# cmusphinx/pocketsphinx

Hardware: NVIDIA H100
Metric: frames/sec senone-eval+Viterbi (higher is better)
Workload: dtype f32->i16/i32

## Files before the change

pocketsphinx_b200/csrc/psb_api.cu:

```cuda
#include "psb_internal.cuh"

#include <stdarg.h>
#include <stdlib.h>
#include <string.h>

#include <algorithm>
#include <vector>

std::atomic<long long> g_psb_launches{0};
std::atomic<long long> g_psb_bytes_live{0};

static thread_local char g_err[512] = "";

void psb_set_error(const char *fmt, ...)
{
    va_list ap;
    va_start(ap, fmt);
    vsnprintf(g_err, sizeof(g_err), fmt, ap);
    va_end(ap);
}

extern "C" const char *psb_last_error(void) { return g_err; }
extern "C" int psb_abi_version(void) { return PSB_ABI_VERSION; }
extern "C" int64_t psb_kernel_launch_count(void) { return g_psb_launches.load(); }
// ... 126 lines not shown
    PSB_CUDA(cudaSetDevice(device));
    PSB_REQUIRE(!(d->fixed_point && d->kind == PSB_KIND_MS), "fixed-point arithmetic is implemented for ptm and semi-continuous models only");
    std::unique_ptr<psb_model_t> m(new psb_model_t());
    m->device = device;
    m->kind = d->kind; m->n_sen = d->n_sen; m->n_mgau = d->n_mgau; m->n_feat = d->n_feat;
    m->n_density = d->n_density; m->topn = d->topn;
    m->ds_ratio = d->ds_ratio > 0 ? d->ds_ratio : 1;
    m->aw = d->aw != 0 ? d->aw : 1;
    m->sumlen = 0;
    for (int f = 0; f < d->n_feat; ++f) {
        m->featlen[f] = d->featlen[f];
        m->featoff[f] = m->sumlen;
        m->sumlen += d->featlen[f];
    }
    m->K = m->n_mgau * m->n_feat;
    m->mixw_4bit = d->mixw_cb != nullptr;
    m->fixed_point = d->fixed_point != 0;
    m->logadd_ms_size = d->logadd_ms_size;
    m->logadd_ms_zero = d->logadd_ms_zero;
    const bool dev = d->on_device != 0;
    const cudaMemcpyKind to_dev = dev ? cudaMemcpyDeviceToDevice : cudaMemcpyHostToDevice;
    int rc = build_records(m.get(), d->mean, d->var, d->det, dev);
    if (!rc) rc = upload(m->d_featlen, m->featlen, PSB_MAX_FEAT, false);
    if (!rc) rc = upload(m->d_featoff, m->featoff, PSB_MAX_FEAT, false);
    if (rc) return rc;

    std::vector<int32_t> s2c(m->n_sen);
    if (cudaMemcpy(s2c.data(), d->sen2cb, m->n_sen * sizeof(int32_t),
                   dev ? cudaMemcpyDeviceToHost : cudaMemcpyHostToHost) != cudaSuccess) {
        psb_set_error("copying sen2cb failed");
        return PSB_ERR_CUDA;
    }
    std::vector<uint16_t> s2c16(m->n_sen);
    for (int i = 0; i < m->n_sen; ++i) {
        PSB_REQUIRE(s2c[i] >= 0 && s2c[i] < m->n_mgau, "sen2cb[%d] = %d out of range", i, s2c[i]);
        s2c16[i] = (uint16_t)s2c[i];
    }
    {
        const int nq = (m->n_sen + 3) / 4;
        std::vector<int16_t> quadcb(nq, -1);
        std::vector<int32_t> bsen;
        for (int q = 0; q < nq; ++q) {
            const int s0 = 4 * q;
            bool uni = s0 + 3 < m->n_sen && m->n_mgau <= 32767;
            for (int i = 1; uni && i < 4; ++i) uni = s2c[s0 + i] == s2c[s0];
            if (uni) quadcb[q] = (int16_t)s2c[s0];
            else for (int i = 0; i < 4 && s0 + i < m->n_sen; ++i) bsen.push_back(s0 + i);
        }
        m->n_bsen = (int)bsen.size();
        if ((rc = upload(m->d_quadcb, quadcb.data(), nq, false)) || (rc = upload(m->d_bsen, bsen.data(), bsen.size(), false)))
            return rc;
    }
    m->sen_is_cb = m->n_mgau == m->n_sen;
    for (int i = 0; m->sen_is_cb && i < m->n_sen; ++i) m->sen_is_cb = s2c[i] == i;
    if ((rc = upload(m->d_sen2cb, s2c16.data(), m->n_sen, false)) || (rc = upload(m->d_sen2cb32, s2c.data(), m->n_sen, false)))
        return rc;

    if (m->kind == PSB_KIND_MS) {
        m->mixw_row = m->n_sen;
        m->mixw_stride = m->n_sen;
        rc = upload(m->d_mixw, d->mixw, (size_t)m->n_sen * m->n_feat * m->n_density, dev);
    }
    else {
        m->mixw_row = m->mixw_4bit ? (m->n_sen + 1) / 2 : m->n_sen;
        m->mixw_stride = roundup(m->mixw_row, 128);
        const size_t rows = (size_t)m->n_feat * m->n_density;
        rc = m->d_mixw.reserve(rows * m->mixw_stride);
        if (!rc && (cudaMemset(m->d_mixw, 0, rows * m->mixw_stride) != cudaSuccess ||
                    cudaMemcpy2D(m->d_mixw, m->mixw_stride, d->mixw, m->mixw_row, m->mixw_row, rows, to_dev) != cudaSuccess)) {
            psb_set_error("uploading mixture weights failed: %s", cudaGetErrorString(cudaGetLastError()));
            rc = PSB_ERR_CUDA;
        }
    }
    if (!rc && m->mixw_4bit) rc = upload(m->d_mixw_cb, d->mixw_cb, 16, dev);
    if (!rc && d->logadd8) {
        rc = m->d_logadd8.reserve(PSB_LOGADD8_N);
        if (!rc && (cudaMemset(m->d_logadd8, 0, PSB_LOGADD8_N) != cudaSuccess ||
                    cudaMemcpy(m->d_logadd8, d->logadd8, 256, to_dev) != cudaSuccess)) {
            psb_set_error("uploading the log-add table failed: %s", cudaGetErrorString(cudaGetLastError()));
            rc = PSB_ERR_CUDA;
        }
        else if (!rc) {
            uint8_t t[256];
            if (cudaMemcpy(t, m->d_logadd8, 256, cudaMemcpyDeviceToHost) == cudaSuccess)
                for (int i = 0; i < 256; ++i) m->logadd8_max = std::max<int>(m->logadd8_max, t[i]);
        }
    }
    if (rc) return rc;
    PSB_REQUIRE(m->kind == PSB_KIND_MS || d->logadd8, "logadd8 table required for ptm/semi models");
    if (m->kind == PSB_KIND_MS) {
        PSB_REQUIRE(d->logadd_ms && d->logadd_ms_size > 0, "logadd_ms table required for ms models");
        rc = upload(m->d_logadd_ms, d->logadd_ms, (size_t)d->logadd_ms_size, dev);
        if (rc) return rc;
    }
    if (d->topn_beam) {
        uint8_t tb[PSB_MAX_FEAT] = {0};
        if (cudaMemcpy(tb, d->topn_beam, m->n_feat, dev ? cudaMemcpyDeviceToHost : cudaMemcpyHostToHost) != cudaSuccess)
            return PSB_ERR_CUDA;
        for (int f = 0; f < m->n_feat; ++f) {
            m->topn_beam[f] = tb[f];
            if (tb[f]) m->has_topn_beam = true;
        }
    }
    int32_t tb[PSB_MAX_FEAT] = {0};
    for (int f = 0; f < m->n_feat; ++f) tb[f] = m->has_topn_beam ? m->topn_beam[f] : 0;
    rc = upload(m->d_topn_beam, tb, PSB_MAX_FEAT, false);
    if (rc) return rc;
    *out = m.release();
    return PSB_OK;
}

extern "C" void psb_model_free(psb_model_t *m)
{
    if (!m) return;
    cudaSetDevice(m->device);
    delete m;
}

extern "C" int psb_model_update_gaussians(psb_model_t *m, const float *mean, const float *var, const float *det)
{
    PSB_REQUIRE(m && mean && var && det, "psb_model_update_gaussians: null argument");
    PSB_CUDA(cudaSetDevice(m->device));
    PSB_CUDA(cudaDeviceSynchronize());
    return build_records(m, mean, var, det, false);
}

extern "C" int psb_model_n_sen(const psb_model_t *m) { return m ? m->n_sen : 0; }
extern "C" int psb_model_device(const psb_model_t *m) { return m ? m->device : -1; }


extern "C" int psb_batch_create(psb_model_t *m, int32_t max_utts, int64_t max_frames, psb_batch_t **out)
{
    PSB_REQUIRE(m && out && max_utts > 0 && max_frames > 0, "psb_batch_create: bad argument");
    const char *v = getenv("PSB_TOPN_VARIANT"), *impl = getenv("PSB_TC_IMPL");
    PSB_REQUIRE(!v || !strcmp(v, "6"),
                "psb_batch_create: PSB_TOPN_VARIANT=%s; the top-N kernel now follows from the model (the only accepted value is 6)", v);
    PSB_REQUIRE(!impl || !strcmp(impl, "wgmma"), "psb_batch_create: PSB_TC_IMPL=%s; the only accepted value is wgmma", impl);
    PSB_CUDA(cudaSetDevice(m->device));
    std::unique_ptr<psb_batch_t> b(new psb_batch_t());
    b->m = m;
    b->max_utts = max_utts;
    b->max_frames = max_frames;
    {
        const char *p = getenv("PSB_PIPELINE");
        b->n_pipe = p ? atoi(p) : 0;
        if (b->n_pipe < 0) b->n_pipe = 0;
        if (b->n_pipe > 8) b->n_pipe = 8;
    }
    cudaError_t e = b->stream.create();
    for (int i = 0; i < 4 && e == cudaSuccess; ++i) e = b->ev[i].create();
    for (int i = 0; i < 2 && e == cudaSuccess; ++i) e = b->tev[i].create();
    if (e == cudaSuccess) e = b->fork_ev.create(cudaEventDisableTiming);
    if (e == cudaSuccess) e = b->join_ev.create(cudaEventDisableTiming);
    if (e != cudaSuccess) {
        psb_set_error("psb_batch_create: %s", cudaGetErrorString(e));
        return PSB_ERR_CUDA;
    }
    int rc = b->d_feats.reserve((size_t)max_frames * m->sumlen);
    if (!rc) rc = b->d_senscr.reserve((size_t)max_frames * m->n_sen);
    if (!rc && m->kind != PSB_KIND_MS) rc = b->topn.reserve((size_t)max_frames * m->K);
    if (rc) return rc;
    b->d_topn = b->topn;
    *out = b.release();
    return PSB_OK;
}

extern "C" void psb_batch_free(psb_batch_t *b)
{
// ... 270 lines not shown
```

pocketsphinx_b200/csrc/psb_internal.cuh:

```cuda
#pragma once

#include <cuda_runtime.h>
#include <stdint.h>
#include <stdio.h>

#include <atomic>
#include <memory>
#include <string>
#include <vector>

#include "../../include/psb200.h"
#include "psb_mem.cuh"

#define PSB_SENSCR_SHIFT 10
#define PSB_MAX_NEG_ASCR 96
#define PSB_TMAT_WORST (-255)
#define PSB_BAD_SSID 0xffff
#define PSB_LOGADD8_N 512

void psb_set_error(const char *fmt, ...);
extern std::atomic<long long> g_psb_launches;

__device__ __forceinline__ float2 psb_fadd2_rn(float2 a, float2 b) { return make_float2(__fadd_rn(a.x, b.x), __fadd_rn(a.y, b.y)); }
__device__ __forceinline__ float2 psb_fmul2_rn(float2 a, float2 b) { return make_float2(__fmul_rn(a.x, b.x), __fmul_rn(a.y, b.y)); }

inline int psb_sm_count(int device)
{
    int n = 1;
    cudaDeviceGetAttribute(&n, cudaDevAttrMultiProcessorCount, device);
    return n;
}

#define PSB_CUDA(call)                                                                   \
    do {                                                                                 \
        cudaError_t e__ = (call);                                                        \
        if (e__ != cudaSuccess) {                                                        \
            psb_set_error("%s:%d: %s -> %s", __FILE__, __LINE__, #call,                  \
                          cudaGetErrorString(e__));                                      \
            return PSB_ERR_CUDA;                                                         \
        }                                                                                \
    } while (0)

#define PSB_LAUNCH_CHECK()                                                               \
    do {                                                                                 \
        g_psb_launches.fetch_add(1, std::memory_order_relaxed);                          \
        cudaError_t e__ = cudaGetLastError();                                            \
        if (e__ != cudaSuccess) {                                                        \
            psb_set_error("%s:%d: kernel launch -> %s", __FILE__, __LINE__,              \
                          cudaGetErrorString(e__));                                      \
            return PSB_ERR_CUDA;                                                         \
        }                                                                                \
    } while (0)

#define PSB_REQUIRE(cond, ...)                                                           \
    do {                                                                                 \
        if (!(cond)) {                                                                   \
            psb_set_error(__VA_ARGS__);                                                  \
            return PSB_ERR_ARG;                                                          \
        }                                                                                \
    } while (0)

static inline int psb_check_utt_off(const char *fn, const int32_t *utt_off, int32_t n_utt)
{
    PSB_REQUIRE(utt_off[0] == 0, "%s: utt_off[0] must be 0", fn);
    for (int u = 0; u < n_utt; ++u)
        PSB_REQUIRE(utt_off[u + 1] >= utt_off[u], "%s: utt_off not monotone at %d", fn, u);
    return PSB_OK;
}

static inline int roundup(int x, int m) { return (x + m - 1) / m * m; }

static inline int rec_floats(int featlen) { return roundup(1 + 2 * featlen, 4); }

struct psb_model_s {
    int device;
    int kind, n_sen, n_mgau, n_feat, n_density, topn, ds_ratio, aw;
    int featlen[PSB_MAX_FEAT], featoff[PSB_MAX_FEAT], sumlen;
    int K;
    bool mixw_4bit;
    bool fixed_point;
    int mixw_row;
    int mixw_stride;
    int logadd_ms_size, logadd_ms_zero;
    DevBuf<float> d_rec;
    std::vector<size_t> rec_off;
    DevBuf<size_t> d_rec_off;
    DevBuf<float> d_rec2;
    DevBuf<size_t> d_rec2_off;
    DevBuf<uint8_t> d_mixw;
    DevBuf<uint8_t> d_mixw_cb;
    DevBuf<uint16_t> d_sen2cb;
    DevBuf<int32_t> d_sen2cb32;
    bool sen_is_cb;
    DevBuf<int16_t> d_quadcb;
    DevBuf<int32_t> d_bsen;
    int n_bsen;
    int logadd8_max;
    DevBuf<uint8_t> d_logadd8;
    DevBuf<uint32_t> d_logadd_ms;
    DevBuf<float> d_msT, d_msdetT;
    DevBuf<int32_t> d_featlen, d_featoff;
    uint8_t topn_beam[PSB_MAX_FEAT];
    DevBuf<int32_t> d_topn_beam;
    bool has_topn_beam;
    bool tc_ok;
    DevBuf<float> d_tc_wumma, d_tc_cen, d_tc_bnd;
};

struct psb_batch_s {
    psb_model_t *m;
    Stream stream;
    int max_utts;
    long long max_frames;
    DevBuf<float> d_feats;
    DevBuf<int16_t> d_senscr;
    DevBuf<float> d_featT;
    DevBuf<int4> topn;
    int4 *d_topn;
    DevBuf<int32_t> d_tab;
    HostBuf<int32_t> h_tab;
    Event ev[4];
    Event tev[2];
    long long last_frames;
    DevBuf<float2> d_semi_dist;
    DevBuf<int32_t> d_uttoff;
    DevBuf<unsigned> d_tc_flags; size_t tc_flag_words;
    DevBuf<float> d_tc_check;
    int tc_last_tpc;
    long long tc_last_ctas;
    DevBuf<uint4> d_tc_items; DevBuf<unsigned> d_tc_nitems; unsigned tc_item_cap;
    DevBuf<int32_t> d_best, d_pen;
    DevBuf<int32_t> d_off;
    DevBuf<unsigned char> d_msdist;
    DevBuf<int32_t> d_msbest;
    std::vector<std::unique_ptr<psb_batch_t>> kids;
    Event fork_ev, join_ev;
    int n_pipe;
    bool last_pipelined;
    int last_kids;
    HostBuf<int32_t> h_off;
};

cudaStream_t psb_batch_stream(psb_batch_t *b);
int psb_phoneloop_launch(psb_phoneloop_t *p, const int16_t *d_senscr, const int32_t *d_utt_off, int32_t n_utt,
                         int32_t *d_best, int32_t *d_pen, psb_hmm_t *d_final, psb_hmm_t *d_trace, cudaStream_t st);
int psb_phoneloop_n_phones(const psb_phoneloop_t *p);
int psb_launch_ptm_batch(psb_batch_t *b, const float *d_feats, const int32_t *utt_off,
                         int32_t n_utt, int16_t *d_senscr);
int psb_tc_prepare(psb_model_t *m, const float *hm, const float *hv, const float *hd);
bool psb_tc_usable(const psb_model_t *m);
int psb_launch_ptm_tc(psb_batch_t *b, const float *d_feats, const int32_t *utt_off, int32_t n_utt, const int32_t *d_klist,
                      const int32_t *d_featoff);
int psb_ms_score_one(psb_model_t *m, cudaStream_t st, const float *d_feat, void *d_dist, int32_t *d_best,
                     int16_t *d_senscr, const int32_t *d_list, int n_items);
size_t psb_ms_dist_bytes(const psb_model_t *m);
int psb_launch_ms_batch(psb_batch_t *b, const float *d_feats, const int32_t *utt_off, int32_t n_utt, int16_t *d_senscr);
```

pocketsphinx_b200/csrc/psb_ptm.cu:

```cuda
#include "psb_gau.cuh"
#include "psb_internal.cuh"

#include <algorithm>
#include <numeric>

namespace {

constexpr int TOPN = 4;
constexpr int TOPN_WARPS = 4;
constexpr int MAX_NDW = 8;

__device__ __forceinline__ int fx_mul(int a, int b)
{
    return (int)(unsigned)(((long long)a * (long long)b) >> 12);
}
__device__ __forceinline__ int fx_gmmsub(int a, int b)
{
    return b < 0 ? INT_MIN : (int)((unsigned)a - (unsigned)b);
}
template <int FL, bool SEMI>
__device__ __forceinline__ int gau_dist_fx(const float4 *__restrict__ r, const float (&x)[FL], int *dmin)
{
    constexpr int RECF = (1 + 2 * FL + 3) / 4 * 4;
    int rr[RECF];
// ... 735 lines not shown
            int fden = w0 + (int)nv.x;
            fden = logadd8(tab, fden, w1 + (int)nv.y);
            fden = logadd8(tab, fden, w2 + (int)nv.z);
            fden = logadd8(tab, fden, w3 + (int)nv.w);
            ascore += fden;
        }
        best = min(best, ascore);
        asc[s] = (int16_t)ascore;
    }
    best = __reduce_min_sync(0xffffffffu, best);
    if ((tid & 31) == 0) red[tid >> 5] = best;
    __syncthreads();
    if (tid < 32) {
        int v = tid < (int)(blockDim.x >> 5) ? red[tid] : 0x7fffffff;
        v = __reduce_min_sync(0xffffffffu, v);
        if (tid == 0) red[0] = v;
    }
    __syncthreads();
    best = red[0];
    int16_t *dst = senscr + frame * n_sen;
    for (int s = tid; s < n_sen; s += blockDim.x)
        dst[s] = (int16_t)(asc[s] - best);
}

template <bool FOURBIT>
__global__ void __launch_bounds__(256)
semi_senone_kernel(const int4 *__restrict__ topn, const uint8_t *__restrict__ mixw,
                   const uint8_t *__restrict__ mixw_cb, const uint8_t *__restrict__ logadd_tab,
                   int16_t *__restrict__ senscr, int n_sen, int n_feat, int nd, int mixw_stride)
{
    extern __shared__ int smem_i[];
    uint4 *rowoff = reinterpret_cast<uint4 *>(smem_i);
    uint4 *nsc = rowoff + n_feat;
    uint8_t *tab = reinterpret_cast<uint8_t *>(nsc + n_feat);
    uint8_t *cb16 = tab + PSB_LOGADD8_N;
    __shared__ int cnt[PSB_MAX_FEAT];
    const long long frame = blockIdx.x;
    const int tid = threadIdx.x;
    for (int i = tid; i < PSB_LOGADD8_N; i += blockDim.x) tab[i] = logadd_tab[i];
    if (FOURBIT && tid < 16) cb16[tid] = mixw_cb[tid];
    if (tid < n_feat) {
        const int4 r = topn[frame * n_feat + tid];
        const unsigned cwb = (unsigned)r.y, eb = (unsigned)r.z;
        unsigned ro[TOPN], nv[TOPN];
#pragma unroll
        for (int j = 0; j < TOPN; ++j) {
            ro[j] = ((unsigned)tid * nd + ((cwb >> (8 * j)) & 0xff)) * (unsigned)mixw_stride;
            nv[j] = (eb >> (8 * j)) & 0xff;
        }
        rowoff[tid] = make_uint4(ro[0], ro[1], ro[2], ro[3]);
        nsc[tid] = make_uint4(nv[0], nv[1], nv[2], nv[3]);
        cnt[tid] = r.x;
    }
    __syncthreads();
    const int s = blockIdx.y * blockDim.x + tid;
    if (s >= n_sen) return;
    int16_t acc = 0;
    if (!FOURBIT || s < (n_sen & ~1)) {
        for (int f = 0; f < n_feat; ++f) {
            const uint4 ro = rowoff[f], nv = nsc[f];
            const unsigned rr[TOPN] = {ro.x, ro.y, ro.z, ro.w}, vv[TOPN] = {nv.x, nv.y, nv.z, nv.w};
            const int n = cnt[f];
            int tmp = 0;
#pragma unroll
            for (int k = 0; k < TOPN; ++k) {
                if (k == 0 || k < n) {
                    int w;
                    if (FOURBIT) {
                        const int b = mixw[rr[k] + (unsigned)(s >> 1)];
                        w = cb16[(s & 1) ? b >> 4 : b & 0x0f];
                    }
                    else
                        w = mixw[rr[k] + (unsigned)s];
                    const int v = w + (int)vv[k];
                    tmp = k == 0 ? v : logadd8(tab, tmp, v);
                }
            }
            acc = (int16_t)(acc + tmp);
        }
    }
    senscr[frame * n_sen + s] = acc;
}

__global__ void __launch_bounds__(512)
ptm_senone4_kernel(const int4 *__restrict__ topn, const uint8_t *__restrict__ mixw,
                   const uint16_t *__restrict__ sen2cb, const int16_t *__restrict__ quadcb,
                   const int32_t *__restrict__ bsen, int n_bsen, const uint8_t *__restrict__ logadd_tab,
                   int16_t *__restrict__ senscr, int n_sen, int n_feat, int nd, int K, int mixw_stride)
{
    extern __shared__ int smem_i[];
    uint4 *rowoff = reinterpret_cast<uint4 *>(smem_i);
    uint4 *nsc = rowoff + K;
    uint4 *nvp = nsc + K;
    int *norm = reinterpret_cast<int *>(nvp + K);
    int *red = norm + 8;
    uint8_t *tab = reinterpret_cast<uint8_t *>(red + 32);
    int16_t *asc = reinterpret_cast<int16_t *>(tab + PSB_LOGADD8_N + 16);
    const long long frame = blockIdx.x;
    const int tid = threadIdx.x;

    for (int i = tid; i < PSB_LOGADD8_N; i += blockDim.x) tab[i] = logadd_tab[i];
    if (tid < n_feat) norm[tid] = PSB_WORST_SCORE;
    __syncthreads();
    int4 r = make_int4(0, 0, 0, 0);
    if (tid < K) {
        r = topn[frame * K + tid];
        atomicMax(&norm[tid % n_feat], r.x);
    }
    __syncthreads();
    if (tid < K) {
        const int f = tid % n_feat;
        const int base = norm[f] - r.x;
        const unsigned eb = (unsigned)r.z, cwb = (unsigned)r.y;
        unsigned ro[TOPN], nv[TOPN];
#pragma unroll
        for (int j = 0; j < TOPN; ++j) {
            int v = base + (int)((eb >> (8 * j)) & 0xff);
            nv[j] = (unsigned)(v > PSB_MAX_NEG_ASCR ? PSB_MAX_NEG_ASCR : v);
            ro[j] = ((unsigned)f * nd + ((cwb >> (8 * j)) & 0xff)) * (unsigned)mixw_stride;
        }
        rowoff[tid] = make_uint4(ro[0], ro[1], ro[2], ro[3]);
        nsc[tid] = make_uint4(nv[0], nv[1], nv[2], nv[3]);
        nvp[tid] = make_uint4((nv[0] + SEN_BIAS) * 0x10001u, (nv[1] + SEN_BIAS) * 0x10001u,
                              (nv[2] + SEN_BIAS) * 0x10001u, (nv[3] + SEN_BIAS) * 0x10001u);
    }
    __syncthreads();

    int best = 0x7fffffff;
    const int n_quads = (n_sen + 3) >> 2;
    for (int q = tid; q < n_quads; q += blockDim.x) {
        const int c = quadcb[q];
        if (c < 0) continue;
        const int s0 = q << 2, i0 = c * n_feat;
        const uint8_t *mw = mixw + s0;
        unsigned acc01 = 0u, acc23 = 0u;
        for (int f = 0; f < n_feat; ++f) {
            const uint4 ro = rowoff[i0 + f], nv = nvp[i0 + f];
            const unsigned w0 = *reinterpret_cast<const unsigned *>(mw + ro.x);
            const unsigned w1 = *reinterpret_cast<const unsigned *>(mw + ro.y);
            const unsigned w2 = *reinterpret_cast<const unsigned *>(mw + ro.z);
            const unsigned w3 = *reinterpret_cast<const unsigned *>(mw + ro.w);
            unsigned x01 = __byte_perm(w0, 0u, 0x4140) + nv.x;
            unsigned x23 = __byte_perm(w0, 0u, 0x4342) + nv.x;
#define PSB_LADD2(x, w, sel, nvj)                                                               \
            {                                                                                   \
                const unsigned y = __byte_perm(w, 0u, sel);                                     \
                const unsigned mn = __viaddmin_u16x2(y, nvj, x);                                \
                const unsigned mx = __viaddmax_u16x2(y, nvj, x);                                \
                const unsigned d = mx - mn;                                                     \
                const unsigned t = (unsigned)tab[d & 0xffffu] | ((unsigned)tab[d >> 16] << 16); \
                x = mn - t;                                                                     \
            }
            PSB_LADD2(x01, w1, 0x4140, nv.y) PSB_LADD2(x23, w1, 0x4342, nv.y)
            PSB_LADD2(x01, w2, 0x4140, nv.z) PSB_LADD2(x23, w2, 0x4342, nv.z)
            PSB_LADD2(x01, w3, 0x4140, nv.w) PSB_LADD2(x23, w3, 0x4342, nv.w)
#undef PSB_LADD2
            acc01 += x01;
            acc23 += x23;
        }
        const int unbias = n_feat * SEN_BIAS;
        const int a0 = (int)(acc01 & 0xffffu) - unbias, a1 = (int)(acc01 >> 16) - unbias;
        const int a2 = (int)(acc23 & 0xffffu) - unbias, a3 = (int)(acc23 >> 16) - unbias;
        best = min(min(best, a0), min(min(a1, a2), a3));
        *reinterpret_cast<short4 *>(asc + s0) = make_short4((short)a0, (short)a1, (short)a2, (short)a3);
    }
    for (int i = tid; i < n_bsen; i += blockDim.x) {
        const int s = bsen[i];
        const int i0 = (int)sen2cb[s] * n_feat;
        const uint8_t *mw = mixw + s;
        int ascore = 0;
        for (int f = 0; f < n_feat; ++f) {
            const uint4 ro = rowoff[i0 + f], nv = nsc[i0 + f];
            int fden = mw[ro.x] + (int)nv.x;
            fden = logadd8(tab, fden, mw[ro.y] + (int)nv.y);
            fden = logadd8(tab, fden, mw[ro.z] + (int)nv.z);
            fden = logadd8(tab, fden, mw[ro.w] + (int)nv.w);
            ascore += fden;
        }
        best = min(best, ascore);
        asc[s] = (int16_t)ascore;
    }
    best = __reduce_min_sync(0xffffffffu, best);
    if ((tid & 31) == 0) red[tid >> 5] = best;
    __syncthreads();
    if (tid < 32) {
        int v = tid < (int)(blockDim.x >> 5) ? red[tid] : 0x7fffffff;
        v = __reduce_min_sync(0xffffffffu, v);
        if (tid == 0) red[0] = v;
    }
    __syncthreads();
    best = red[0];
    int16_t *dst = senscr + frame * n_sen;
    for (int s = tid; s < n_sen; s += blockDim.x)
        dst[s] = (int16_t)(asc[s] - best);
}

template <int FL>
int launch_topn2(psb_batch_t *b, const int32_t *d_klist, int n_k, const GroupTabs &tabs, int n_groups,
                 const int32_t *d_featoff)
{
    psb_model_t *m = b->m;
    constexpr int RECF2 = (2 + 4 * FL + 3) / 4 * 4;
    size_t smem = (size_t)(m->n_density / 2) * RECF2 * sizeof(float);
    auto kern = ptm_topn2_kernel<FL>;
    PSB_CUDA(cudaFuncSetAttribute(kern, cudaFuncAttributeMaxDynamicSharedMemorySize, (int)smem));
    dim3 grid(n_k, (n_groups + TOPN_WARPS - 1) / TOPN_WARPS);
    kern<<<grid, TOPN_WARPS * 32, smem, b->stream>>>(m->d_rec2, m->d_rec2_off, d_klist, b->d_featT, tabs, b->d_topn, n_groups,
                                                    m->n_density, m->n_feat, m->sumlen, d_featoff, m->K, m->ds_ratio,
                                                    m->d_topn_beam);
    PSB_LAUNCH_CHECK();
    return PSB_OK;
}

template <int FL>
int launch_topnq(psb_batch_t *b, const int32_t *d_klist, int n_k, const GroupTabs &tabs, int n_groups,
                 const int32_t *d_featoff)
{
    psb_model_t *m = b->m;
    constexpr int RECF2 = (2 + 4 * FL + 3) / 4 * 4;
    const size_t smem = (size_t)(m->n_density / 2) * RECF2 * sizeof(float) + (size_t)QCAP * TOPN_WARPS * 32 * sizeof(float);
    auto kern = ptm_topnq_kernel<FL>;
    PSB_CUDA(cudaFuncSetAttribute(kern, cudaFuncAttributeMaxDynamicSharedMemorySize, (int)smem));
    dim3 grid(n_k, (n_groups + TOPN_WARPS - 1) / TOPN_WARPS);
    kern<<<grid, TOPN_WARPS * 32, smem, b->stream>>>(m->d_rec2, m->d_rec2_off, d_klist, b->d_featT, tabs, b->d_topn, n_groups,
                                                    m->n_density, m->n_feat, m->sumlen, d_featoff, m->K, m->ds_ratio);
    PSB_LAUNCH_CHECK();
    return PSB_OK;
}

template <int FL, bool SEMI>
int launch_topn(psb_batch_t *b, const int32_t *d_klist, int n_k, const GroupTabs &tabs, int n_groups,
                const int32_t *d_featoff)
{
    psb_model_t *m = b->m;
    if constexpr (FL <= 16) {
        if (!m->fixed_point) {
            if constexpr (SEMI) return launch_topn2<FL>(b, d_klist, n_k, tabs, n_groups, d_featoff);
            else return launch_topnq<FL>(b, d_klist, n_k, tabs, n_groups, d_featoff);
        }
    }
    auto kern = ptm_topn_kernel<FL, SEMI, true>;
    if constexpr (FL > 16) {
        if (!m->fixed_point) kern = ptm_topn_kernel<FL, SEMI, false>;
    }
    size_t smem = (size_t)m->n_density * rec_floats(FL) * sizeof(float);
    PSB_CUDA(cudaFuncSetAttribute(kern, cudaFuncAttributeMaxDynamicSharedMemorySize, (int)smem));
    const int warps = (long long)n_k * ((n_groups + TOPN_WARPS - 1) / TOPN_WARPS) >= 4 * psb_sm_count(m->device) ? TOPN_WARPS : 1;
    dim3 grid(n_k, (n_groups + warps - 1) / warps);
    kern<<<grid, warps * 32, smem, b->stream>>>(m->d_rec, m->d_rec_off, d_klist, b->d_featT, tabs, b->d_topn, n_groups,
                                               m->n_density, m->n_feat, m->sumlen, d_featoff, m->K, m->ds_ratio,
                                               m->d_topn_beam);
    PSB_LAUNCH_CHECK();
    return PSB_OK;
}

__global__ void __launch_bounds__(512)
semi_senone4_kernel(const int4 *__restrict__ topn, const uint8_t *__restrict__ mixw,
                    const uint8_t *__restrict__ logadd_tab, int16_t *__restrict__ senscr, int n_sen, int n_feat, int nd,
                    int mixw_stride)
{
    __shared__ uint4 rowoff[PSB_MAX_FEAT], nvp[PSB_MAX_FEAT], nsc[PSB_MAX_FEAT];
    __shared__ int cnt[PSB_MAX_FEAT];
    __shared__ uint8_t tab[PSB_LOGADD8_N];
    const long long frame = blockIdx.x;
    const int tid = threadIdx.x;
    for (int i = tid; i < PSB_LOGADD8_N; i += blockDim.x) tab[i] = logadd_tab[i];
    if (tid < n_feat) {
        const int4 r = topn[frame * n_feat + tid];
        const unsigned cwb = (unsigned)r.y, eb = (unsigned)r.z;
        unsigned ro[TOPN], nv[TOPN];
#pragma unroll
        for (int j = 0; j < TOPN; ++j) {
            ro[j] = ((unsigned)tid * nd + ((cwb >> (8 * j)) & 0xff)) * (unsigned)mixw_stride;
            nv[j] = (eb >> (8 * j)) & 0xff;
        }
        rowoff[tid] = make_uint4(ro[0], ro[1], ro[2], ro[3]);
        nsc[tid] = make_uint4(nv[0], nv[1], nv[2], nv[3]);
        nvp[tid] = make_uint4((nv[0] + SEN_BIAS) * 0x10001u, (nv[1] + SEN_BIAS) * 0x10001u,
                              (nv[2] + SEN_BIAS) * 0x10001u, (nv[3] + SEN_BIAS) * 0x10001u);
        cnt[tid] = r.x;
    }
    __syncthreads();
    int16_t *dst = senscr + frame * n_sen;
    const int n_quads = n_sen >> 2;
    for (int q = tid; q < n_quads; q += blockDim.x) {
        const int s0 = q << 2;
        const uint8_t *mw = mixw + s0;
        short a0 = 0, a1 = 0, a2 = 0, a3 = 0;
        for (int f = 0; f < n_feat; ++f) {
            const uint4 ro = rowoff[f], nv = nvp[f];
            const int n = cnt[f];
            const unsigned w0 = *reinterpret_cast<const unsigned *>(mw + ro.x);
            unsigned x01 = __byte_perm(w0, 0u, 0x4140) + nv.x, x23 = __byte_perm(w0, 0u, 0x4342) + nv.x;
#define PSB_LADD2(x, w, sel, nvj)                                                               \
            {                                                                                   \
                const unsigned y = __byte_perm(w, 0u, sel);                                     \
                const unsigned mn = __viaddmin_u16x2(y, nvj, x);                                \
                const unsigned mx = __viaddmax_u16x2(y, nvj, x);                                \
                const unsigned d = mx - mn;                                                     \
                const unsigned t = (unsigned)tab[d & 0xffffu] | ((unsigned)tab[d >> 16] << 16); \
                x = mn - t;                                                                     \
            }
            if (n > 1) {
                const unsigned w1 = *reinterpret_cast<const unsigned *>(mw + ro.y);
                PSB_LADD2(x01, w1, 0x4140, nv.y) PSB_LADD2(x23, w1, 0x4342, nv.y)
            }
            if (n > 2) {
                const unsigned w2 = *reinterpret_cast<const unsigned *>(mw + ro.z);
                PSB_LADD2(x01, w2, 0x4140, nv.z) PSB_LADD2(x23, w2, 0x4342, nv.z)
            }
            if (n > 3) {
                const unsigned w3 = *reinterpret_cast<const unsigned *>(mw + ro.w);
                PSB_LADD2(x01, w3, 0x4140, nv.w) PSB_LADD2(x23, w3, 0x4342, nv.w)
            }
#undef PSB_LADD2
            a0 = (short)(a0 + (int)(x01 & 0xffffu) - SEN_BIAS);
            a1 = (short)(a1 + (int)(x01 >> 16) - SEN_BIAS);
            a2 = (short)(a2 + (int)(x23 & 0xffffu) - SEN_BIAS);
            a3 = (short)(a3 + (int)(x23 >> 16) - SEN_BIAS);
        }
        if ((((uintptr_t)(dst + s0)) & 7) == 0)
            *reinterpret_cast<short4 *>(dst + s0) = make_short4(a0, a1, a2, a3);
        else { dst[s0] = a0; dst[s0 + 1] = a1; dst[s0 + 2] = a2; dst[s0 + 3] = a3; }
    }
    for (int s = (n_quads << 2) + tid; s < n_sen; s += blockDim.x) {
        int16_t acc = 0;
        for (int f = 0; f < n_feat; ++f) {
            const uint4 ro = rowoff[f], nv = nsc[f];
            const unsigned rr[TOPN] = {ro.x, ro.y, ro.z, ro.w}, vv[TOPN] = {nv.x, nv.y, nv.z, nv.w};
            const int n = cnt[f];
            int tmp = 0;
#pragma unroll
            for (int k = 0; k < TOPN; ++k)
                if (k == 0 || k < n) {
                    const int v = mixw[rr[k] + (unsigned)s] + (int)vv[k];
                    tmp = k == 0 ? v : logadd8(tab, tmp, v);
                }
            acc = (int16_t)(acc + tmp);
        }
        dst[s] = acc;
    }
}

}

int psb_launch_ptm_batch(psb_batch_t *b, const float *d_feats, const int32_t *utt_off, int32_t n_utt,
                         int16_t *d_senscr)
{
    psb_model_t *m = b->m;
    PSB_REQUIRE(m->kind == PSB_KIND_PTM || m->kind == PSB_KIND_SEMI, "psb_launch_ptm_batch: model is neither PTM nor semi-continuous");
    const bool semi = m->kind == PSB_KIND_SEMI;
    PSB_REQUIRE(m->topn == TOPN, "tied-mixture batch kernels are built for -topn 4 (got %d)", m->topn);
    PSB_REQUIRE(m->n_density % 32 == 0 && m->n_density <= 32 * MAX_NDW,
                "PTM batch kernels need n_density in {32..256, multiple of 32} (got %d)", m->n_density);
    const long long total = utt_off[n_utt];
    PSB_REQUIRE(n_utt <= b->max_utts && total <= b->max_frames, "batch too large for this psb_batch_t");
    b->last_frames = total;
    if (total == 0 || n_utt == 0) return PSB_OK;
    const int D = m->sumlen, K = m->K;

    std::vector<int> perm(n_utt);
    std::iota(perm.begin(), perm.end(), 0);
    std::stable_sort(perm.begin(), perm.end(), [&](int a, int c) {
        return utt_off[a + 1] - utt_off[a] > utt_off[c + 1] - utt_off[c];
    });
    const int n_groups = (n_utt + 31) / 32;
    size_t n32 = (size_t)n_groups * 64 + n_groups + K + PSB_MAX_FEAT;
    n32 = (n32 + 1) & ~(size_t)1;
    size_t need = n32 + 2 * (size_t)(2 * n_groups + 1);
    int rc = b->d_tab.reserve(need, need);
    if (!rc) rc = b->h_tab.reserve(need, need);
    if (rc) return rc;
    int32_t *lane_len = b->h_tab, *lane_off = lane_len + n_groups * 32, *grp_maxT = lane_off + n_groups * 32;
    int32_t *klist = grp_maxT + n_groups, *featoff = klist + K;
    long long *grp_base = reinterpret_cast<long long *>(b->h_tab + n32), *warp_base = grp_base + n_groups;
    long long featT_floats = 0, items = 0;
    for (int g = 0; g < n_groups; ++g) {
        int mx = 0;
        for (int l = 0; l < 32; ++l) {
            int idx = g * 32 + l;
            if (idx < n_utt) {
                int u = perm[idx];
                lane_len[idx] = utt_off[u + 1] - utt_off[u];
                lane_off[idx] = utt_off[u];
                mx = std::max(mx, lane_len[idx]);
            }
            else { lane_len[idx] = 0; lane_off[idx] = 0; }
        }
        grp_maxT[g] = mx;
        grp_base[g] = featT_floats;
        warp_base[g] = items;
        featT_floats += (long long)mx * D * 32;
        items += mx;
    }
    warp_base[n_groups] = items;
    for (int f = 0; f < PSB_MAX_FEAT; ++f) featoff[f] = f < m->n_feat ? m->featoff[f] : 0;
    if ((rc = b->d_featT.reserve((size_t)featT_floats, (size_t)featT_floats >> 3))) return rc;
    std::vector<std::vector<int>> byfl;
    std::vector<int> fls;
    for (int f = 0; f < m->n_feat; ++f) {
        size_t i = std::find(fls.begin(), fls.end(), m->featlen[f]) - fls.begin();
        if (i == fls.size()) { fls.push_back(m->featlen[f]); byfl.emplace_back(); }
        for (int cb = 0; cb < m->n_mgau; ++cb) byfl[i].push_back(cb * m->n_feat + f);
    }
    {
        int pos = 0;
        for (auto &v : byfl) for (int k : v) klist[pos++] = k;
    }
    PSB_CUDA(cudaMemcpyAsync(b->d_tab, b->h_tab, need * sizeof(int32_t), cudaMemcpyHostToDevice, b->stream));
    GroupTabs tabs;
    tabs.lane_len = b->d_tab;
    tabs.lane_off = b->d_tab + n_groups * 32;
    tabs.grp_maxT = b->d_tab + n_groups * 64;
    const int32_t *d_klist = b->d_tab + n_groups * 64 + n_groups, *d_featoff = d_klist + K;
    tabs.grp_base = reinterpret_cast<const long long *>(b->d_tab + n32);
    const long long *d_warp_base = tabs.grp_base + n_groups;

    const bool use_tc = !semi && psb_tc_usable(m);
    PSB_CUDA(cudaEventRecord(b->ev[0], b->stream));
    if (!use_tc) {
        int warps = 8;
        while (warps > 1 && (size_t)warps * 32 * (D + 1) * sizeof(float) > 48 * 1024) warps >>= 1;
        size_t smem = (size_t)warps * 32 * (D + 1) * sizeof(float);
        PSB_REQUIRE(smem <= 48 * 1024, "feature vectors of %d floats are too long for transpose_feats_kernel", D);
// ... 13 lines not shown
        const size_t need_d = (size_t)K * total * m->n_density;
        if ((rc = b->d_semi_dist.reserve(need_d, need_d / 8)) || (rc = b->d_uttoff.reserve((size_t)n_utt + 1, 64))) return rc;
        PSB_CUDA(cudaMemcpyAsync(b->d_uttoff, utt_off, ((size_t)n_utt + 1) * sizeof(int32_t), cudaMemcpyHostToDevice, b->stream));
        PSB_REQUIRE(total <= 0x7fffffffLL, "too many frames for one launch");
        int pos = 0;
        for (size_t i = 0; i < fls.size(); ++i) {
            const int n_k = (int)byfl[i].size();
            const dim3 grid((unsigned)total, (unsigned)n_k);
            switch (fls[i]) {
#define CASE(FL) case FL: semi_dist_kernel<FL><<<grid, roundup(m->n_density, 32), 0, b->stream>>>(                     \
                    m->d_rec, m->d_rec_off, d_klist + pos, d_feats, b->d_semi_dist, total, m->n_density, m->n_feat, D, d_featoff); break;
                CASE(13) CASE(12) CASE(24) CASE(3) CASE(39) CASE(1) CASE(2) CASE(4) CASE(8) CASE(16) CASE(26) CASE(32)
#undef CASE
            default:
                psb_set_error("no semi_dist_kernel instantiation for stream length %d", fls[i]);
                return PSB_ERR_ARG;
            }
            PSB_LAUNCH_CHECK();
            pos += n_k;
        }
        const int warps = 4;
        const unsigned blocks = (unsigned)(((long long)n_utt * K + warps - 1) / warps);
        if (m->n_density == 256)
            semi_scan_kernel<8><<<blocks, warps * 32, 0, b->stream>>>(b->d_semi_dist, b->d_uttoff, n_utt, K, total, 256, m->ds_ratio, m->d_topn_beam, b->d_topn);
        else if (m->n_density == 128)
            semi_scan_kernel<4><<<blocks, warps * 32, 0, b->stream>>>(b->d_semi_dist, b->d_uttoff, n_utt, K, total, 128, m->ds_ratio, m->d_topn_beam, b->d_topn);
        else
            semi_scan_kernel<2><<<blocks, warps * 32, 0, b->stream>>>(b->d_semi_dist, b->d_uttoff, n_utt, K, total, 64, m->ds_ratio, m->d_topn_beam, b->d_topn);
        PSB_LAUNCH_CHECK();
    }
    else {
        int pos = 0;
        for (size_t i = 0; i < fls.size(); ++i) {
            int n_k = (int)byfl[i].size(), rc;
            switch (fls[i]) {
#define CASE(FL) case FL: rc = semi ? launch_topn<FL, true>(b, d_klist + pos, n_k, tabs, n_groups, d_featoff) \
                                   : launch_topn<FL, false>(b, d_klist + pos, n_k, tabs, n_groups, d_featoff); break;
                CASE(13) CASE(12) CASE(24) CASE(3) CASE(39) CASE(1) CASE(2) CASE(4) CASE(8) CASE(16) CASE(26) CASE(32)
#undef CASE
            default:
                psb_set_error("no ptm_topn_kernel instantiation for stream length %d", fls[i]);
                return PSB_ERR_ARG;
            }
            if (rc) return rc;
            pos += n_k;
        }
    }
    PSB_CUDA(cudaEventRecord(b->ev[2], b->stream));
    if (semi) {
        size_t smem = (size_t)K * 32 + PSB_LOGADD8_N + 16;
        PSB_REQUIRE(K <= 512, "semi_senone_kernel handles at most 512 streams (got %d)", K);
        const int threads = 256;
        dim3 grid((m->n_sen + threads - 1) / threads, (unsigned)total);
        PSB_REQUIRE(total <= 65535LL * 32768, "too many frames for one launch");
        if (!m->mixw_4bit && (TOPN - 1) * m->logadd8_max < SEN_BIAS && m->mixw_stride % 4 == 0 &&
            m->n_feat <= PSB_MAX_FEAT)
            semi_senone4_kernel<<<(unsigned)total, 512, 0, b->stream>>>(b->d_topn, m->d_mixw, m->d_logadd8, d_senscr, m->n_sen,
                                                                      m->n_feat, m->n_density, m->mixw_stride);
        else if (m->mixw_4bit)
            semi_senone_kernel<true><<<dim3((unsigned)total, (m->n_sen + threads - 1) / threads), threads, smem, b->stream>>>(
                b->d_topn, m->d_mixw, m->d_mixw_cb, m->d_logadd8, d_senscr, m->n_sen, m->n_feat, m->n_density, m->mixw_stride);
        else
            semi_senone_kernel<false><<<dim3((unsigned)total, (m->n_sen + threads - 1) / threads), threads, smem, b->stream>>>(
                b->d_topn, m->d_mixw, m->d_mixw_cb, m->d_logadd8, d_senscr, m->n_sen, m->n_feat, m->n_density, m->mixw_stride);
        (void)grid;
        PSB_LAUNCH_CHECK();
    }
    else {
        size_t smem = (size_t)K * 32 + 8 * 4 + 32 * 4 + PSB_LOGADD8_N + 16 + (size_t)m->n_sen * 2;
        PSB_REQUIRE(K <= 512, "ptm_senone_kernel handles at most 512 (codebook, stream) pairs (got %d)", K);
        PSB_REQUIRE((size_t)m->n_feat * m->n_density * m->mixw_stride < (1ull << 32), "mixture-weight table too large for 32-bit offsets");
        if (m->mixw_4bit) {
            PSB_CUDA(cudaFuncSetAttribute(ptm_senone_kernel<true>, cudaFuncAttributeMaxDynamicSharedMemorySize, (int)smem));
            ptm_senone_kernel<true><<<(unsigned)total, 512, smem, b->stream>>>(
                b->d_topn, m->d_mixw, m->d_mixw_cb, m->d_sen2cb, m->d_logadd8, d_senscr, m->n_sen, m->n_feat,
                m->n_density, K, m->mixw_stride);
        }
        else if ((TOPN - 1) * m->logadd8_max >= SEN_BIAS) {
            PSB_CUDA(cudaFuncSetAttribute(ptm_senone_kernel<false>, cudaFuncAttributeMaxDynamicSharedMemorySize, (int)smem));
            ptm_senone_kernel<false><<<(unsigned)total, 512, smem, b->stream>>>(
                b->d_topn, m->d_mixw, m->d_mixw_cb, m->d_sen2cb, m->d_logadd8, d_senscr, m->n_sen, m->n_feat,
                m->n_density, K, m->mixw_stride);
        }
        else {
            const int n_quads = (m->n_sen + 3) / 4;
            const int iters = (n_quads + 511) / 512;
            const int threads = std::min(512, std::max(std::max(256, roundup(K, 32)), roundup((n_quads + iters - 1) / iters, 32)));
            const size_t smem4 = smem + 8 + (size_t)K * 16;
            PSB_CUDA(cudaFuncSetAttribute(ptm_senone4_kernel, cudaFuncAttributeMaxDynamicSharedMemorySize, (int)smem4));
            ptm_senone4_kernel<<<(unsigned)total, threads, smem4, b->stream>>>(
                b->d_topn, m->d_mixw, m->d_sen2cb, m->d_quadcb, m->d_bsen, m->n_bsen, m->d_logadd8, d_senscr, m->n_sen,
                m->n_feat, m->n_density, K, m->mixw_stride);
        }
        PSB_LAUNCH_CHECK();
    }
    PSB_CUDA(cudaEventRecord(b->ev[3], b->stream));
    return PSB_OK;
}
```

Measured before the change: 12.78 million.

## Keep PTM senone quad scores in registers and add templated senone4 variants

The quad-packed PTM senone kernel becomes a template over stream count and option flags. When the senone count fits in three quads per thread, the default launch picks a variant that holds the packed accumulators in registers. It then subtracts the block best and writes them straight to global memory, skipping the shared-memory round trip and the final rescan. It also sets launch bounds to allow more resident blocks, and adds an optional clamped log-add table plus timing-probe variants behind a compile flag. Risks are higher register pressure and extra template instantiations.

```diff
diff --git a/pocketsphinx_b200/csrc/psb_api.cu b/pocketsphinx_b200/csrc/psb_api.cu
--- a/pocketsphinx_b200/csrc/psb_api.cu
+++ b/pocketsphinx_b200/csrc/psb_api.cu
@@ -232,8 +232,15 @@
         }
         else if (!rc) {
             uint8_t t[256];
-            if (cudaMemcpy(t, m->d_logadd8, 256, cudaMemcpyDeviceToHost) == cudaSuccess)
-                for (int i = 0; i < 256; ++i) m->logadd8_max = std::max<int>(m->logadd8_max, t[i]);
+            if (cudaMemcpy(t, m->d_logadd8, 256, cudaMemcpyDeviceToHost) != cudaSuccess) {
+                psb_set_error("reading back the log-add table failed: %s", cudaGetErrorString(cudaGetLastError()));
+                rc = PSB_ERR_CUDA;
+            }
+            else
+                for (int i = 0; i < 256; ++i) {
+                    m->logadd8_max = std::max<int>(m->logadd8_max, t[i]);
+                    if (t[i]) m->logadd8_zero = i + 1;
+                }
         }
     }
     if (rc) return rc;
diff --git a/pocketsphinx_b200/csrc/psb_internal.cuh b/pocketsphinx_b200/csrc/psb_internal.cuh
--- a/pocketsphinx_b200/csrc/psb_internal.cuh
+++ b/pocketsphinx_b200/csrc/psb_internal.cuh
@@ -96,6 +96,7 @@
     DevBuf<int32_t> d_bsen;
     int n_bsen;
     int logadd8_max;
+    int logadd8_zero;
     DevBuf<uint8_t> d_logadd8;
     DevBuf<uint32_t> d_logadd_ms;
     DevBuf<float> d_msT, d_msdetT;
diff --git a/pocketsphinx_b200/csrc/psb_ptm.cu b/pocketsphinx_b200/csrc/psb_ptm.cu
--- a/pocketsphinx_b200/csrc/psb_ptm.cu
+++ b/pocketsphinx_b200/csrc/psb_ptm.cu
@@ -841,12 +841,57 @@
     senscr[frame * n_sen + s] = acc;
 }
 
-__global__ void __launch_bounds__(512)
+enum { SEN4_CLAMP = 1, SEN4_REGS = 2, SEN4_PROBE_TAB = 4, SEN4_PROBE_ROW = 8 };
+constexpr int SEN4_QPT = 3;
+
+template <int OPT>
+__device__ __forceinline__ unsigned sen4_ladd2(const uint8_t *tab, unsigned zz, unsigned x, unsigned y, unsigned nvj)
+{
+    const unsigned mn = __viaddmin_u16x2(y, nvj, x);
+    const unsigned mx = __viaddmax_u16x2(y, nvj, x);
+    unsigned d = mx - mn;
+    if (OPT & SEN4_CLAMP) d = __vminu2(d, zz);
+    const unsigned t = (OPT & SEN4_PROBE_TAB) ? 0x00010001u
+                                              : (unsigned)tab[d & 0xffffu] | ((unsigned)tab[d >> 16] << 16);
+    return mn - t;
+}
+
+template <int NF, int OPT>
+__device__ __forceinline__ void sen4_quad(const uint8_t *__restrict__ mw, const uint4 *rowoff, const uint4 *nvp,
+                                          const uint8_t *tab, unsigned zz, int i0, int n_feat, unsigned &acc01,
+                                          unsigned &acc23)
+{
+    acc01 = acc23 = 0u;
+    for (int f = 0; f < (NF ? NF : n_feat); ++f) {
+        uint4 ro = rowoff[i0 + f];
+        const uint4 nv = nvp[i0 + f];
+        if (OPT & SEN4_PROBE_ROW) ro = make_uint4(0u, 0u, 0u, 0u);
+        const unsigned w0 = *reinterpret_cast<const unsigned *>(mw + ro.x);
+        const unsigned w1 = *reinterpret_cast<const unsigned *>(mw + ro.y);
+        const unsigned w2 = *reinterpret_cast<const unsigned *>(mw + ro.z);
+        const unsigned w3 = *reinterpret_cast<const unsigned *>(mw + ro.w);
+        unsigned x01 = __byte_perm(w0, 0u, 0x4140) + nv.x;
+        unsigned x23 = __byte_perm(w0, 0u, 0x4342) + nv.x;
+        x01 = sen4_ladd2<OPT>(tab, zz, x01, __byte_perm(w1, 0u, 0x4140), nv.y);
+        x23 = sen4_ladd2<OPT>(tab, zz, x23, __byte_perm(w1, 0u, 0x4342), nv.y);
+        x01 = sen4_ladd2<OPT>(tab, zz, x01, __byte_perm(w2, 0u, 0x4140), nv.z);
+        x23 = sen4_ladd2<OPT>(tab, zz, x23, __byte_perm(w2, 0u, 0x4342), nv.z);
+        x01 = sen4_ladd2<OPT>(tab, zz, x01, __byte_perm(w3, 0u, 0x4140), nv.w);
+        x23 = sen4_ladd2<OPT>(tab, zz, x23, __byte_perm(w3, 0u, 0x4342), nv.w);
+        acc01 += x01;
+        acc23 += x23;
+    }
+}
+
+template <int NF, int OPT>
+__global__ void __launch_bounds__(512, 4)
 ptm_senone4_kernel(const int4 *__restrict__ topn, const uint8_t *__restrict__ mixw,
                    const uint16_t *__restrict__ sen2cb, const int16_t *__restrict__ quadcb,
-                   const int32_t *__restrict__ bsen, int n_bsen, const uint8_t *__restrict__ logadd_tab,
-                   int16_t *__restrict__ senscr, int n_sen, int n_feat, int nd, int K, int mixw_stride)
-{
+                   const int32_t *__restrict__ bsen, int n_bsen, const uint8_t *__restrict__ logadd_tab, int tab_z,
+                   int16_t *__restrict__ senscr, int n_sen, int n_feat_arg, int nd, int K, int mixw_stride)
+{
+    constexpr bool CLAMP = OPT & SEN4_CLAMP, REGS = OPT & SEN4_REGS;
+    const int n_feat = NF ? NF : n_feat_arg;
     extern __shared__ int smem_i[];
     uint4 *rowoff = reinterpret_cast<uint4 *>(smem_i);
     uint4 *nsc = rowoff + K;
@@ -857,8 +902,9 @@
     int16_t *asc = reinterpret_cast<int16_t *>(tab + PSB_LOGADD8_N + 16);
     const long long frame = blockIdx.x;
     const int tid = threadIdx.x;
-
-    for (int i = tid; i < PSB_LOGADD8_N; i += blockDim.x) tab[i] = logadd_tab[i];
+    const unsigned zz = (unsigned)tab_z * 0x10001u;
+
+    for (int i = tid; i < (CLAMP ? tab_z + 1 : PSB_LOGADD8_N); i += blockDim.x) tab[i] = logadd_tab[i];
     if (tid < n_feat) norm[tid] = PSB_WORST_SCORE;
     __syncthreads();
     int4 r = make_int4(0, 0, 0, 0);
@@ -885,44 +931,36 @@
     }
     __syncthreads();
 
-    int best = 0x7fffffff;
     const int n_quads = (n_sen + 3) >> 2;
-    for (int q = tid; q < n_quads; q += blockDim.x) {
-        const int c = quadcb[q];
-        if (c < 0) continue;
-        const int s0 = q << 2, i0 = c * n_feat;
-        const uint8_t *mw = mixw + s0;
-        unsigned acc01 = 0u, acc23 = 0u;
-        for (int f = 0; f < n_feat; ++f) {
-            const uint4 ro = rowoff[i0 + f], nv = nvp[i0 + f];
-            const unsigned w0 = *reinterpret_cast<const unsigned *>(mw + ro.x);
-            const unsigned w1 = *reinterpret_cast<const unsigned *>(mw + ro.y);
-            const unsigned w2 = *reinterpret_cast<const unsigned *>(mw + ro.z);
-            const unsigned w3 = *reinterpret_cast<const unsigned *>(mw + ro.w);
-            unsigned x01 = __byte_perm(w0, 0u, 0x4140) + nv.x;
-            unsigned x23 = __byte_perm(w0, 0u, 0x4342) + nv.x;
-#define PSB_LADD2(x, w, sel, nvj)                                                               \
-            {                                                                                   \
-                const unsigned y = __byte_perm(w, 0u, sel);                                     \
-                const unsigned mn = __viaddmin_u16x2(y, nvj, x);                                \
-                const unsigned mx = __viaddmax_u16x2(y, nvj, x);                                \
-                const unsigned d = mx - mn;                                                     \
-                const unsigned t = (unsigned)tab[d & 0xffffu] | ((unsigned)tab[d >> 16] << 16); \
-                x = mn - t;                                                                     \
-            }
-            PSB_LADD2(x01, w1, 0x4140, nv.y) PSB_LADD2(x23, w1, 0x4342, nv.y)
-            PSB_LADD2(x01, w2, 0x4140, nv.z) PSB_LADD2(x23, w2, 0x4342, nv.z)
-            PSB_LADD2(x01, w3, 0x4140, nv.w) PSB_LADD2(x23, w3, 0x4342, nv.w)
-#undef PSB_LADD2
-            acc01 += x01;
-            acc23 += x23;
-        }
-        const int unbias = n_feat * SEN_BIAS;
-        const int a0 = (int)(acc01 & 0xffffu) - unbias, a1 = (int)(acc01 >> 16) - unbias;
-        const int a2 = (int)(acc23 & 0xffffu) - unbias, a3 = (int)(acc23 >> 16) - unbias;
-        best = min(min(best, a0), min(min(a1, a2), a3));
-        *reinterpret_cast<short4 *>(asc + s0) = make_short4((short)a0, (short)a1, (short)a2, (short)a3);
-    }
+    const int unbias = n_feat * SEN_BIAS;
+    unsigned bmin = 0xffffffffu;
+    unsigned keep[REGS ? 2 * SEN4_QPT : 1];
+    if (REGS) {
+#pragma unroll
+        for (int j = 0; j < SEN4_QPT; ++j) {
+            const int q = tid + j * (int)blockDim.x;
+            const int c = q < n_quads ? quadcb[q] : -1;
+            unsigned acc01 = 0xffffffffu, acc23 = 0xffffffffu;
+            if (c >= 0) {
+                sen4_quad<NF, OPT>(mixw + (q << 2), rowoff, nvp, tab, zz, c * n_feat, n_feat, acc01, acc23);
+                bmin = __vminu2(bmin, __vminu2(acc01, acc23));
+            }
+            keep[2 * j] = acc01;
+            keep[2 * j + 1] = acc23;
+        }
+    }
+    else {
+        for (int q = tid; q < n_quads; q += blockDim.x) {
+            const int c = quadcb[q];
+            if (c < 0) continue;
+            unsigned acc01, acc23;
+            sen4_quad<NF, OPT>(mixw + (q << 2), rowoff, nvp, tab, zz, c * n_feat, n_feat, acc01, acc23);
+            bmin = __vminu2(bmin, __vminu2(acc01, acc23));
+            const unsigned sub = (unsigned)unbias * 0x10001u;
+            *reinterpret_cast<uint2 *>(asc + (q << 2)) = make_uint2(__vsub2(acc01, sub), __vsub2(acc23, sub));
+        }
+    }
+    int best = bmin == 0xffffffffu ? 0x7fffffff : min((int)(bmin & 0xffffu), (int)(bmin >> 16)) - unbias;
     for (int i = tid; i < n_bsen; i += blockDim.x) {
         const int s = bsen[i];
         const int i0 = (int)sen2cb[s] * n_feat;
@@ -931,9 +969,16 @@
         for (int f = 0; f < n_feat; ++f) {
             const uint4 ro = rowoff[i0 + f], nv = nsc[i0 + f];
             int fden = mw[ro.x] + (int)nv.x;
-            fden = logadd8(tab, fden, mw[ro.y] + (int)nv.y);
-            fden = logadd8(tab, fden, mw[ro.z] + (int)nv.z);
-            fden = logadd8(tab, fden, mw[ro.w] + (int)nv.w);
+            if (CLAMP) {
+                fden = min(fden, mw[ro.y] + (int)nv.y) - tab[min(abs(fden - (mw[ro.y] + (int)nv.y)), tab_z)];
+                fden = min(fden, mw[ro.z] + (int)nv.z) - tab[min(abs(fden - (mw[ro.z] + (int)nv.z)), tab_z)];
+                fden = min(fden, mw[ro.w] + (int)nv.w) - tab[min(abs(fden - (mw[ro.w] + (int)nv.w)), tab_z)];
+            }
+            else {
+                fden = logadd8(tab, fden, mw[ro.y] + (int)nv.y);
+                fden = logadd8(tab, fden, mw[ro.z] + (int)nv.z);
+                fden = logadd8(tab, fden, mw[ro.w] + (int)nv.w);
+            }
             ascore += fden;
         }
         best = min(best, ascore);
@@ -950,8 +995,31 @@
     __syncthreads();
     best = red[0];
     int16_t *dst = senscr + frame * n_sen;
-    for (int s = tid; s < n_sen; s += blockDim.x)
-        dst[s] = (int16_t)(asc[s] - best);
+    if (REGS) {
+        const unsigned sub = ((unsigned)(unbias + best) & 0xffffu) * 0x10001u;
+        const bool al4 = (reinterpret_cast<uintptr_t>(dst) & 3) == 0;
+#pragma unroll
+        for (int j = 0; j < SEN4_QPT; ++j) {
+            if ((keep[2 * j] & keep[2 * j + 1]) == 0xffffffffu) continue;
+            const int s0 = (tid + j * (int)blockDim.x) << 2;
+            const unsigned v01 = __vsub2(keep[2 * j], sub), v23 = __vsub2(keep[2 * j + 1], sub);
+            if (al4) {
+                *reinterpret_cast<unsigned *>(dst + s0) = v01;
+                *reinterpret_cast<unsigned *>(dst + s0 + 2) = v23;
+            }
+            else {
+                dst[s0] = (int16_t)v01; dst[s0 + 1] = (int16_t)(v01 >> 16);
+                dst[s0 + 2] = (int16_t)v23; dst[s0 + 3] = (int16_t)(v23 >> 16);
+            }
+        }
+        for (int i = tid; i < n_bsen; i += blockDim.x) {
+            const int s = bsen[i];
+            dst[s] = (int16_t)(asc[s] - best);
+        }
+    }
+    else
+        for (int s = tid; s < n_sen; s += blockDim.x)
+            dst[s] = (int16_t)(asc[s] - best);
 }
 
 template <int FL>
@@ -1099,6 +1167,30 @@
         }
         dst[s] = acc;
     }
+}
+
+template <int NF, int OPT>
+int launch_senone4(psb_batch_t *b, const int4 *records, int16_t *d_senscr, long long total)
+{
+    psb_model_t *m = b->m;
+    const int K = m->K, n_quads = (m->n_sen + 3) / 4, iters = (n_quads + 511) / 512;
+    PSB_REQUIRE(NF == 0 || NF == m->n_feat, "ptm_senone4_kernel<%d>: the model has %d streams", NF, m->n_feat);
+    PSB_REQUIRE(!(OPT & SEN4_REGS) || iters <= SEN4_QPT, "ptm_senone4_kernel: %d senones exceed %d quads per thread", m->n_sen, SEN4_QPT);
+    const int threads = std::min(512, std::max(std::max(256, roundup(K, 32)), roundup((n_quads + iters - 1) / iters, 32)));
+    const size_t smem = (size_t)K * 48 + 8 * 4 + 32 * 4 + PSB_LOGADD8_N + 16 + 8 + (size_t)m->n_sen * 2;
+    auto kern = ptm_senone4_kernel<NF, OPT>;
+    PSB_CUDA(cudaFuncSetAttribute(kern, cudaFuncAttributeMaxDynamicSharedMemorySize, (int)smem));
+    kern<<<(unsigned)total, threads, smem, b->stream>>>(records, m->d_mixw, m->d_sen2cb, m->d_quadcb, m->d_bsen, m->n_bsen,
+                                                         m->d_logadd8, m->logadd8_zero, d_senscr, m->n_sen, m->n_feat,
+                                                         m->n_density, K, m->mixw_stride);
+    PSB_LAUNCH_CHECK();
+    return PSB_OK;
+}
+
+int launch_senone4_lib(psb_batch_t *b, const int4 *records, int16_t *d_senscr, long long total)
+{
+    if ((b->m->n_sen + 3) / 4 <= 512 * SEN4_QPT) return launch_senone4<0, SEN4_REGS>(b, records, d_senscr, total);
+    return launch_senone4<0, 0>(b, records, d_senscr, total);
 }
 
 }
@@ -1278,18 +1370,46 @@
                 b->d_topn, m->d_mixw, m->d_mixw_cb, m->d_sen2cb, m->d_logadd8, d_senscr, m->n_sen, m->n_feat,
                 m->n_density, K, m->mixw_stride);
         }
-        else {
-            const int n_quads = (m->n_sen + 3) / 4;
-            const int iters = (n_quads + 511) / 512;
-            const int threads = std::min(512, std::max(std::max(256, roundup(K, 32)), roundup((n_quads + iters - 1) / iters, 32)));
-            const size_t smem4 = smem + 8 + (size_t)K * 16;
-            PSB_CUDA(cudaFuncSetAttribute(ptm_senone4_kernel, cudaFuncAttributeMaxDynamicSharedMemorySize, (int)smem4));
-            ptm_senone4_kernel<<<(unsigned)total, threads, smem4, b->stream>>>(
-                b->d_topn, m->d_mixw, m->d_sen2cb, m->d_quadcb, m->d_bsen, m->n_bsen, m->d_logadd8, d_senscr, m->n_sen,
-                m->n_feat, m->n_density, K, m->mixw_stride);
-        }
+        else if ((rc = launch_senone4_lib(b, b->d_topn, d_senscr, total)))
+            return rc;
         PSB_LAUNCH_CHECK();
     }
     PSB_CUDA(cudaEventRecord(b->ev[3], b->stream));
     return PSB_OK;
 }
+
+#ifdef PSB_SENONE_CANDIDATES
+extern "C" int psb_senone_candidate_device(psb_batch_t *b, const int4 *records, int16_t *senscr, int32_t variant, float *ms)
+{
+    PSB_REQUIRE(b && senscr && ms && b->m->kind == PSB_KIND_PTM && !b->m->mixw_4bit, "psb_senone_candidate_device: bad argument");
+    PSB_REQUIRE((TOPN - 1) * b->m->logadd8_max < SEN_BIAS, "psb_senone_candidate_device: the add table is too wide for ptm_senone4_kernel");
+    PSB_CUDA(cudaSetDevice(b->m->device));
+    if (!records) records = b->d_topn;
+    const long long total = b->last_frames;
+    PSB_CUDA(cudaEventRecord(b->ev[2], b->stream));
+    int rc;
+    switch (variant) {
+    case 0: rc = launch_senone4_lib(b, records, senscr, total); break;
+    case 1: rc = launch_senone4<0, 0>(b, records, senscr, total); break;
+    case 2: rc = launch_senone4<0, SEN4_CLAMP>(b, records, senscr, total); break;
+    case 3: rc = launch_senone4<3, 0>(b, records, senscr, total); break;
+    case 4: rc = launch_senone4<0, SEN4_REGS>(b, records, senscr, total); break;
+    case 5: rc = launch_senone4<3, SEN4_CLAMP>(b, records, senscr, total); break;
+    case 6: rc = launch_senone4<0, SEN4_CLAMP | SEN4_REGS>(b, records, senscr, total); break;
+    case 7: rc = launch_senone4<3, SEN4_REGS>(b, records, senscr, total); break;
+    case 8: rc = launch_senone4<3, SEN4_CLAMP | SEN4_REGS>(b, records, senscr, total); break;
+    case 9: rc = launch_senone4<0, SEN4_PROBE_TAB>(b, records, senscr, total); break;
+    case 10: rc = launch_senone4<0, SEN4_PROBE_ROW>(b, records, senscr, total); break;
+    case 11: rc = launch_senone4<3, SEN4_CLAMP | SEN4_REGS | SEN4_PROBE_TAB>(b, records, senscr, total); break;
+    case 12: rc = launch_senone4<3, SEN4_CLAMP | SEN4_REGS | SEN4_PROBE_ROW>(b, records, senscr, total); break;
+    default:
+        psb_set_error("psb_senone_candidate_device: no variant %d", variant);
+        return PSB_ERR_ARG;
+    }
+    if (rc) return rc;
+    PSB_CUDA(cudaEventRecord(b->ev[3], b->stream));
+    PSB_CUDA(cudaEventSynchronize(b->ev[3]));
+    PSB_CUDA(cudaEventElapsedTime(ms, b->ev[2], b->ev[3]));
+    return PSB_OK;
+}
+#endif
```

Result: faster. 12.94 million (median of 6 runs) (+1.2%).
